# arpitbansal297/Cold-Diffusion-Models

Hardware: AMD Instinct MI355X
Metric: unet_train_imgs_per_sec (higher is better)
Workload: dtype f32 storage/accumulate; dense-conv GEMM operands bf16x3; 1 GPU; CelebA-128 denoising cold diffusion (BASELINE config 3): Unet(dim=64,(1,2,4,8),ch=3) @128x128, T=200, optimizer step = 2 micro-batches x 32 img (one fused forward / backward pass over all of them: same draws, same gradient sum) + Adam + EMA/10; per_gpu_batch=32, gradient_accumulate_every=2, parallelism=single

## Files before the change

### cold-diffusion-models_amd/csrc/k_conv_rowhalo.hip

```cpp
#include "cdf_conv_sp.h"

template <int W, int BN, int NS = 3, int NCH = 2, int BM = 256>
__global__ void __launch_bounds__(512, 1) conv_igemm_rowhalo_stream_kernel(SpxArgs a) {
    constexpr int WM = BM / 64, WN = 8 / WM, NW = 8, BK = 32, RE = CDF_SP_RE, MT = BM / WM / 32, NB = 3;
    static_assert(BM == 256 && WM * WN == 8 && MT == 2, "8 waves (4 x 2) of 64-row tiles");
    static_assert(NCH % 2 == 0, "an even number of tap-row groups per tile returns the pipeline to row buffer 0");
    using L = RowHaloLayout<W, BN, BM>;
    using Segs = typename L::Segs;
    constexpr int EROWS = L::EROWS, CP = L::CP;
    constexpr int TH = L::TH, HW2 = L::HW2, RH = L::RH;
    constexpr int TAG = Segs::PER_WAVE;
    constexpr int NT = BN / WN / 32;
    constexpr int SB = BN / 16 / NW;
    static_assert(SB * NW * 16 == BN || BN == 64, "B tile must split into 16-row segments");
    constexpr int SBI = BN == 64 ? 1 : SB;
    constexpr int PLANE_A = L::PLANE_A, PLANE_B = L::PLANE_B;
    CDF_DYN_SMEM(smem_raw);
    unsigned short* smem = (unsigned short*)smem_raw;
    float* const cs = (float*)(smem + L::OFF_CS);

    const int tid = threadIdx.x, lane = tid & 63, wave = __builtin_amdgcn_readfirstlane(tid >> 6);
    const int wm = wave / WN, wn = wave % WN;
    const int M = a.B * a.QH * a.QW;
    const int tiles_n = (a.Cout + BN - 1) / BN, tiles_m = M / BM, ntiles = tiles_m * tiles_n;
    const CdfPhase& ph = a.ph[0];
    const int tpi = a.H / TH;

    const int srow = cdf_dma_row(lane), q8 = cdf_dma_col(lane);
    int a_seg[TAG], a_ry[TAG], a_x[TAG];
#pragma unroll
    for (int q = 0; q < TAG; ++q) {
        const int g = a_seg[q] = Segs::seg(wave, q);
        const int r = g * 16 + srow;
        a_ry[q] = r < RH ? r / HW2 : -(1 << 20);
        a_x[q] = r - (r / HW2) * HW2 - 1;
    }
    auto fetch_a = [&](int img, int y0, int c, int dy, int buf) {
        unsigned short* base = smem + L::a_off(buf);
#pragma unroll
        for (int q = 0; q < TAG; ++q) {
            const int y = y0 + a_ry[q] + dy;
            const bool ok = img >= 0 && (unsigned)y < (unsigned)a.H && (unsigned)a_x[q] < (unsigned)W;
            const size_t off = ((size_t)(((ok ? img : 0) * a.H + (ok ? y : 0)) * W + (ok ? a_x[q] : 0))) * (unsigned)a.ldx + (unsigned)(c * BK + q8);
            unsigned short* seg = base + a_seg[q] * 16 * RE;
            CDF_GLDS16_K(ok ? a.x_hi + off : a.zero, seg);
            if constexpr (NS == 3) CDF_GLDS16_K(ok ? a.x_lo + off : a.zero, seg + PLANE_A);
        }
    };
    auto fetch_b = [&](int tile_n, int c, int wi, int stage) {
        unsigned short* st = smem + L::b_off(stage);
#pragma unroll
        for (int p = 0; p < SBI; ++p) {
            const int seg = BN == 64 ? (wave & 3) : wave * SB + p;
            const size_t woff = cdf_w_off(wi, a.Cout, cdf_w_row(tile_n * BN + seg * 16 + srow, a.Cout), a.ldk, c * BK + q8);
            CDF_GLDS16_K(a.w_hi + woff, st + seg * 16 * RE);
            if constexpr (NS == 3) CDF_GLDS16_K(a.w_lo + woff, st + PLANE_B + seg * 16 * RE);
        }
    };
    constexpr int NPL = NS == 3 ? 2 : 1;
    constexpr int PB = NPL * SBI, PAG = NPL * TAG;

    const int half = lane >> 5, l31 = lane & 31;
    int row0[MT];
#pragma unroll
    for (int i = 0; i < MT; ++i) {
        const int pix = wm * (BM / WM) + i * 32 + l31;
        const int py = pix / W, px = pix - py * W;
        row0[i] = py * HW2 + px + 1;
    }
    const bool late = a.dephase != 0 && wave >= NW / 2;

    auto tile_pos = [&](int v, int& img, int& y0, int& tn, int& tm) {
        if (v < ntiles) {
            const int tile = cdf_xcd_order(v, ntiles);
            tm = tile / tiles_n;
            tn = tile - tm * tiles_n;
            img = tm / tpi;
            y0 = (tm - img * tpi) * TH;
        } else {
            img = -1; y0 = 0; tn = 0; tm = 0;
        }
    };
    int img, y0, tile_n, tile_m;
    int v = blockIdx.x;
    tile_pos(v, img, y0, tile_n, tile_m);
    const bool fast_epi = cdf_epi_tile_ok<BM, BN>(a, M) && cdf_epi_family_ok(a.epi, NS == 1);
    fetch_a(img, y0, 0, ph.dy[0], 0);
    fetch_b(tile_n, 0, ph.wi[0], 0);
    fetch_b(tile_n, 0, ph.wi[1], 1);
    CDF_WAIT_DMA_LEAVE(PB);
    CDF_LDS_BARRIER();

    while (img >= 0) {
        int img_n, y0_n, tile_n_n, tile_m_n;
        tile_pos(v + gridDim.x, img_n, y0_n, tile_n_n, tile_m_n);
        f32x16_t acc[MT][NT];
        cdf_acc_zero(acc);
        bf16x8_v ah[2][MT], al[2][MT], bh[2][NT], bl[2][NT];
        if (late) cdf_frag_zero(ah, al, bh, bl);
        auto mma_frags = [&]() { cdf_mma_tile<NS, MT, NT>(acc, ah, al, bh, bl); };
        int row0t[MT], l31t = l31;
#pragma unroll
        for (int i = 0; i < MT; ++i) row0t[i] = row0[i];
#ifndef CDF_EMU
#pragma unroll
        for (int i = 0; i < MT; ++i) asm volatile("" : "+v"(row0t[i]));
        asm volatile("" : "+v"(l31t));
#endif
        const int swbt = (l31t >> 2) & 3;
#pragma unroll
        for (int g = 0; g < 3; ++g) {
#pragma unroll
            for (int c = 0; c < NCH; ++c) {
#pragma unroll
                for (int i3 = 0; i3 < 3; ++i3) {
                    const int t = 3 * g + i3;
                    const int step = (g * NCH + c) * 3 + i3;
                    const int par = (g * NCH + c) & 1, rd = step % NB;
                    {
                        const int s2 = step + 2, gc2 = (s2 / 3) % (3 * NCH);
                        const bool over = s2 >= 9 * NCH;
                        const int g2 = gc2 / NCH, c2 = gc2 - g2 * NCH;
                        fetch_b(over ? tile_n_n : tile_n, c2, ph.wi[3 * g2 + s2 % 3], s2 % NB);
                    }
                    if (i3 == 0) {
                        const bool lastc = c + 1 == NCH, over = lastc && g == 2;
                        const int nc = lastc ? 0 : c + 1, ng = over ? 0 : (lastc ? g + 1 : g);
                        fetch_a(over ? img_n : img, over ? y0_n : y0, nc, ph.dy[3 * ng], par ^ 1);
                    }
                    int sa_e = L::a_off(par), sb_e = L::b_off(rd);
#ifndef CDF_EMU
                    asm volatile("" : "+s"(sa_e), "+s"(sb_e));
#endif
                    const unsigned short* sa = smem + sa_e;
                    const unsigned short* sb = smem + sb_e;
                    const int dx = ph.dx[t];
                    auto read_frags = [&]() {
#pragma unroll
                        for (int ks = 0; ks < 2; ++ks) {
                            cdf_read_frags_halo<NS, PLANE_A>(ah[ks], al[ks], sa, ks, half, row0t, dx);
                            cdf_read_frags<NS, PLANE_B>(bh[ks], bl[ks], sb, ks, half, wn * (BN / WN) + l31t, swbt);
                        }
                    };
                    cdf_dephased_step(late, read_frags, mma_frags);
                    if (i3 <= 1)
                        CDF_WAIT_DMA_LEAVE(PB + PAG);
                    else
                        CDF_WAIT_DMA_LEAVE(PB);
                    CDF_LDS_BARRIER();
                }
            }
        }
        if (late) mma_frags();
        auto dump = [&](int hp) {
            if ((wm * 64) / EROWS == hp) {
                int base = (wm * 64 - hp * EROWS + 4 * half) * CP + wn * (BN / WN) + l31;
#ifndef CDF_EMU
                asm volatile("" : "+v"(base));
#endif
                cdf_acc_stage(cs + base, CP, 0, 0, acc, 0, 0);
            }
        };
        if (fast_epi) {
            const long long trow = (long long)tile_m * BM;
            cdf_epi_dispatch<NS == 1>(a.epi, [&](auto spec) {
                using E = cdf_epi_fast<BN, EROWS, 512, decltype(spec)>;
                f32x4_t q[E::NR], bs[2];
                cdf_epi_load_bias<BN, 512>(a, bs, trow, tile_n * BN, tid);
                E::load(a, q, trow, tile_n * BN, tid);
                dump(0);
                CDF_LDS_BARRIER();
                E::template finish<true>(a, q, bs, cs, trow, tile_n * BN, tid, trow + EROWS);
                CDF_LDS_BARRIER();
                dump(1);
                CDF_LDS_BARRIER();
                E::template finish<false>(a, q, bs, cs, trow + EROWS, tile_n * BN, tid);
                CDF_LDS_BARRIER();
            });
        } else {
#pragma unroll 1
            for (int hp = 0; hp < 2; ++hp) {
                dump(hp);
                CDF_LDS_BARRIER();
                cdf_epilogue_rows<BN, EROWS, 512>(a, ph, a.y, cs, tile_m * BM + hp * EROWS, tile_n * BN, M, tid, [](int p) { return p; });
                CDF_LDS_BARRIER();
            }
        }
        img = img_n; y0 = y0_n; tile_n = tile_n_n; tile_m = tile_m_n;
        v += gridDim.x;
    }
    CDF_WAIT_DMA_LEAVE(0);
}

template <int NS, int W, int BN>
static int launch_igemm_rowhalo_stream(const SpxArgs& a, int M, hipStream_t s, int reserve, CdfPlan* plan) {
    using L = RowHaloLayout<W, BN>;
    const int tiles = (M / 256) * cdf_cdiv(a.Cout, BN);
#ifdef CDF_EMU
    int ncu = cdf_num_cus() - reserve;
    if (ncu < 1) ncu = 1;
#else
    int ncu = cdf_num_cus() - (reserve + 7) / 8 * 8;
    if (ncu < 8) ncu = 8;
#endif
    const int grid = tiles < ncu ? tiles : ncu;
    if (plan) return cdf_plan_set(plan, CDF_FORM_ROWHALO, 256, BN, a.Cin == 64 ? 2 : 4, 1, W, tiles, grid);
    if (a.Cin == 64)
        CDF_LAUNCH_LDS((conv_igemm_rowhalo_stream_kernel<W, BN, NS, 2>), dim3(grid), dim3(512), L::bytes, s, a);
    else
        CDF_LAUNCH_LDS((conv_igemm_rowhalo_stream_kernel<W, BN, NS, 4>), dim3(grid), dim3(512), L::bytes, s, a);
    return cdf_check_launch("conv_igemm_rowhalo_stream");
}


template <int NS>
static int launch_rowhalo_ns(int W, bool n64, const SpxArgs& a, int M, hipStream_t s, int reserve, CdfPlan* plan) {
#define CDF_ROWHALO_CASE(WW) \
    if (W == WW) return n64 ? launch_igemm_rowhalo_stream<NS, WW, 64>(a, M, s, reserve, plan) : launch_igemm_rowhalo_stream<NS, WW, 128>(a, M, s, reserve, plan);
    CDF_ROWHALO_CASE(128)
#ifdef CDF_EMU
    CDF_ROWHALO_CASE(64) CDF_ROWHALO_CASE(32) CDF_ROWHALO_CASE(16)
#endif
#undef CDF_ROWHALO_CASE
    return CDF_E_UNSUPPORTED;
}

int cdf_launch_igemm_rowhalo(int ns, int W, bool n64, const SpxArgs& a, int M, hipStream_t s, int reserve, CdfPlan* plan) {
    return ns == 3 ? launch_rowhalo_ns<3>(W, n64, a, M, s, reserve, plan) : launch_rowhalo_ns<1>(W, n64, a, M, s, reserve, plan);
}
```

### cold-diffusion-models_amd/csrc/k_conv_spx.hip

```cpp
#include "cdf_conv_sp.h"

template <int BM, int BN, int WM, int WN, int NSTAGE, int OCC = 512 / (64 * WM * WN), int NS = 3>
__global__ void __launch_bounds__(64 * WM * WN, OCC) conv_igemm_spx_kernel(SpxArgs a) {
    constexpr int BK = 32, RE = CDF_SP_RE, NW = WM * WN;
    constexpr int MT = BM / WM / 32, NT = BN / WN / 32;
    constexpr int SA = BM / 16 / NW, SB = BN / 16 / NW;
    static_assert(SA >= 1 && SB >= 1 && SA * NW * 16 == BM && SB * NW * 16 == BN, "tile must split into 16-row segments per wave");
    using L = SpxLayout<BM, BN, NSTAGE>;
    constexpr int PLANE_A = L::PLANE_A, PLANE_B = L::PLANE_B, STAGE = L::STAGE;
    CDF_DYN_SMEM(smem_raw);
    unsigned short* smem = (unsigned short*)smem_raw;

    const int tid = threadIdx.x, lane = tid & 63, wave = __builtin_amdgcn_readfirstlane(tid >> 6);
    const int wm = wave / WN, wn = wave % WN;
    const int M = a.B * a.QH * a.QW;
    const int tiles_n = (a.Cout + BN - 1) / BN, tiles_m = (M + BM - 1) / BM;
    const int tile = cdf_xcd_order(blockIdx.x, tiles_m * tiles_n);
    const int tile_m = tile / tiles_n, tile_n = tile - tile_m * tiles_n;
    const CdfPhase& ph = a.ph[blockIdx.y];

    const int srow = cdf_dma_row(lane), q8 = cdf_dma_col(lane);
    int a_iy0[SA], a_ix0[SA], b_row[SB];
    unsigned a_pix[SA];
#pragma unroll
    for (int p = 0; p < SA; ++p) {
        const int m = tile_m * BM + (wave * SA + p) * 16 + srow;
        if (m < M) {
            const int qx = m % a.QW, t2 = m / a.QW;
            a_iy0[p] = (t2 % a.QH) * a.is;
            a_ix0[p] = qx * a.is;
            a_pix[p] = (unsigned)(((t2 / a.QH) * a.H + a_iy0[p]) * a.W + a_ix0[p]);
        } else {
            a_iy0[p] = -(1 << 28);
            a_ix0[p] = 0;
            a_pix[p] = 0;
        }
    }
#pragma unroll
    for (int p = 0; p < SB; ++p) {
        b_row[p] = cdf_w_row(tile_n * BN + (wave * SB + p) * 16 + srow, a.Cout);
    }
    const int nchunks = (a.Cin + BK - 1) / BK;
    const int ntaps_blk = a.ksplit > 1 ? ph.ntaps / a.ksplit : ph.ntaps;
    const int tap_lo = a.ksplit > 1 ? (int)blockIdx.z * ntaps_blk : 0;
    const int niter = ntaps_blk * nchunks;

    int* tap_lds = (int*)(smem + L::OFF_TAPS);
    if (tid <= CDF_MAX_TAPS) {
        int src = tid + tap_lo;
        if (src > CDF_MAX_TAPS) src = CDF_MAX_TAPS;
        if (a.taprot && tid < 9) {
            const int slot = tid / 3, kx = tid - 3 * slot;
#pragma unroll
            for (int g = 0; g < 3; ++g) {
                const int r = (tile_m + (int)ph.dy[3 * g]) % 3;
                if ((r < 0 ? r + 3 : r) == slot) src = 3 * g + kx;
            }
        }
        tap_lds[tid] = src < ph.ntaps ? (ph.dy[src] & 0xFF) | ((ph.dx[src] & 0xFF) << 8) | ((ph.wi[src] & 0xFF) << 16) : 0;
    }
    CDF_LDS_BARRIER();

    const unsigned short* pa_hi[SA];
    const unsigned short* pa_lo[SA];
    const unsigned short* pb_hi[SB];
    const unsigned short* pb_lo[SB];
    int a_inc[SA];
    const bool ragged = (a.Cin & (BK - 1)) != 0;
    auto retap = [&](int tap) {
        const int tc = tap_lds[tap];
        const int dy = (int)(signed char)(tc & 0xFF), dx = (int)(signed char)((tc >> 8) & 0xFF), wi = (tc >> 16) & 0xFF;
        const int tap_pix = dy * a.W + dx;
#pragma unroll
        for (int p = 0; p < SA; ++p) {
            const unsigned iy = (unsigned)(a_iy0[p] + dy), ix = (unsigned)(a_ix0[p] + dx);
            const bool ok = iy < (unsigned)a.H && ix < (unsigned)a.W && q8 < a.Cin;
            const size_t off = (size_t)(a_pix[p] + (unsigned)tap_pix) * (unsigned)a.ldx + (unsigned)q8;
            pa_hi[p] = ok ? a.x_hi + off : a.zero;
            pa_lo[p] = ok ? a.x_lo + off : a.zero;
            a_inc[p] = ok ? BK : 0;
        }
#pragma unroll
        for (int p = 0; p < SB; ++p) {
            const size_t woff = cdf_w_off(wi, a.Cout, b_row[p], a.ldk, q8);
            pb_hi[p] = a.w_hi + woff;
            pb_lo[p] = a.w_lo + woff;
        }
    };
    int tap = 0, c0 = 0, issued = 0;
    retap(0);
    auto fetch = [&](int buf) {
        unsigned short* st = smem + buf * STAGE;
        const bool cok = !ragged || (c0 + q8) < a.Cin;
#pragma unroll
        for (int p = 0; p < SA; ++p) {
            unsigned short* seg = st + (wave * SA + p) * 16 * RE;
            CDF_GLDS16(cok ? pa_hi[p] : a.zero, seg);
            if constexpr (NS == 3) CDF_GLDS16(cok ? pa_lo[p] : a.zero, seg + PLANE_A);
        }
#pragma unroll
        for (int p = 0; p < SB; ++p) {
            unsigned short* seg = st + L::OFF_B + (wave * SB + p) * 16 * RE;
            CDF_GLDS16(pb_hi[p], seg);
            if constexpr (NS == 3) CDF_GLDS16(pb_lo[p], seg + PLANE_B);
        }
        const bool more = issued + 1 < niter;
        issued += more ? 1 : 0;
        if (more) {
            c0 += BK;
            if (c0 >= a.Cin) {
                c0 = 0;
                ++tap;
                retap(tap);
            } else {
#pragma unroll
                for (int p = 0; p < SA; ++p) {
                    pa_hi[p] += a_inc[p];
                    pa_lo[p] += a_inc[p];
                }
#pragma unroll
                for (int p = 0; p < SB; ++p) {
                    pb_hi[p] += BK;
                    pb_lo[p] += BK;
                }
            }
        }
    };

    f32x16_t acc[MT][NT];
    cdf_acc_zero(acc);

    const int half = lane >> 5, l31 = lane & 31;
    const int sw = (l31 >> 2) & 3;
    constexpr int PIECES = (NS == 3 ? 2 : 1) * (SA + SB);
    int fbuf = 0;
    if (niter > 0) {
#pragma unroll
        for (int d = 0; d < NSTAGE - 1; ++d) {
            fetch(fbuf);
            fbuf = fbuf + 1 == NSTAGE ? 0 : fbuf + 1;
        }
    }
    CDF_WAIT_DMA_LEAVE((NSTAGE - 2) * PIECES);
    CDF_LDS_BARRIER();
    int buf = 0;
    bf16x8_v ah[2][MT], al[2][MT], bh[2][NT], bl[2][NT];
    const bool late = a.dephase != 0 && NW == 8 && wave >= 4;
    if (late) cdf_frag_zero(ah, al, bh, bl);
    auto fetch_read = [&]() {
        fetch(fbuf);
        fbuf = fbuf + 1 == NSTAGE ? 0 : fbuf + 1;
        const unsigned short* sa = smem + buf * STAGE;
        const unsigned short* sb = sa + L::OFF_B;
        buf = buf + 1 == NSTAGE ? 0 : buf + 1;
#pragma unroll
        for (int ks = 0; ks < 2; ++ks) {
            cdf_read_frags<NS, PLANE_A>(ah[ks], al[ks], sa, ks, half, wm * (BM / WM) + l31, sw);
            cdf_read_frags<NS, PLANE_B>(bh[ks], bl[ks], sb, ks, half, wn * (BN / WN) + l31, sw);
        }
    };
    auto mma_frags = [&]() { cdf_mma_tile<NS, MT, NT>(acc, ah, al, bh, bl); };
    for (int it = 0; it < niter; ++it) {
        cdf_dephased_step(late, fetch_read, mma_frags);
        CDF_WAIT_DMA_LEAVE((NSTAGE - 2) * PIECES);
        CDF_LDS_BARRIER();
    }
    if (late) mma_frags();
    CDF_WAIT_DMA_LEAVE(0);
    CDF_LDS_BARRIER();

    if (a.ksplit > 1) {
        RawEpiArgs r;
        r.Cout = a.Cout; r.vec = (a.Cout & 3) == 0 ? 1 : 0; r.os = 1; r.QH = 1; r.QW = 1; r.OH = 1; r.OW = 1; r.ldy = a.ks_ld;
        r.ldp = r.ldm = r.ldr = r.ld_sbias = r.ld_ys = 0; r.act = 0; r.mul_mode = 0; r.accumulate = 0;
        r.bias = nullptr; r.sbias = nullptr; r.pre = nullptr; r.mul = nullptr; r.res = nullptr; r.ys_hi = nullptr; r.ys_lo = nullptr; r.io_bf = 0;
        float* cs = (float*)smem_raw;
        cdf_acc_stage(cs, BN + 8, wm * (BM / WM), wn * (BN / WN), acc, half, l31);
        __syncthreads();
        cdf_epilogue_rows<BN, BM, 64 * WM * WN>(r, ph, a.ks_ws + (size_t)blockIdx.z * M * a.ks_ld, cs, tile_m * BM, tile_n * BN, M, tid,
                                                [](int p) { return p; });
        return;
    }
    cdf_sp_epilogue<BM, BN, WM, WN, NS == 1>(a, ph, acc, (float*)smem_raw, tile_m, tile_n, M, tid);
}

template <int BN>
__global__ void __launch_bounds__(256) conv_splitk_finish_kernel(SpxArgs a) {
    constexpr int BM = 16, CP = BN + 8;
    __shared__ __attribute__((aligned(16))) float cs[BM * CP];
    const int tid = threadIdx.x;
    const int M = a.B * a.QH * a.QW;
    const int tiles_n = (a.Cout + BN - 1) / BN;
    const int tile_m = blockIdx.x / tiles_n, tile_n = blockIdx.x - tile_m * tiles_n;
    constexpr int V = BN / 4;
    const size_t zs = (size_t)M * a.ks_ld;
    for (int e = tid; e < BM * V; e += 256) {
        const int r = e / V, c4 = (e - r * V) * 4;
        const int m = tile_m * BM + r, n = tile_n * BN + c4;
        const bool ok = m < M && n < a.ks_ld;
        const float* p = a.ks_ws + (ok ? (size_t)m * a.ks_ld + n : 0);
        float4 v[CDF_MAX_TAPS];
#pragma unroll
        for (int z = 0; z < CDF_MAX_TAPS; ++z) v[z] = *(const float4*)(p + (z < a.ksplit ? z : 0) * zs);
        float4 sum = make_float4(0.f, 0.f, 0.f, 0.f);
#pragma unroll
        for (int z = 0; z < CDF_MAX_TAPS; ++z)
            if (z < a.ksplit) { sum.x += v[z].x; sum.y += v[z].y; sum.z += v[z].z; sum.w += v[z].w; }
        *(float4*)(cs + r * CP + c4) = ok ? sum : make_float4(0.f, 0.f, 0.f, 0.f);
    }
    __syncthreads();
    cdf_epilogue_rows<BN, BM, 256>(a, a.ph[0], a.y, cs, tile_m * BM, tile_n * BN, M, tid, [](int p) { return p; });
}

extern "C" int cdf_gemm_tuning_default(cdf_gemm_tuning* t) {
    CDF_REQUIRE(t, "cdf_gemm_tuning_default: null pointer");
    *t = kTuneDefault;
    return 0;
}

template <int NS, int BM, int BN, int WM, int WN, int NSTAGE, int OCC = 512 / (64 * WM * WN)>
static int launch_igemm_spx(const SpxArgs& a, int M, hipStream_t s, CdfPlan* plan) {
    using L = SpxLayout<BM, BN, NSTAGE>;
    const int tiles = cdf_cdiv(M, BM) * cdf_cdiv(a.Cout, BN);
    if (plan) return cdf_plan_set(plan, CDF_FORM_SPX, BM, BN, NSTAGE, a.ksplit > 1 ? a.ksplit : 1, 0, tiles, (long long)tiles * a.nphase * (a.ksplit > 1 ? a.ksplit : 1));
    CDF_LAUNCH_LDS((conv_igemm_spx_kernel<BM, BN, WM, WN, NSTAGE, OCC, NS>), dim3(tiles, a.nphase, a.ksplit > 1 ? a.ksplit : 1), dim3(64 * WM * WN), L::bytes, s, a);
    if (a.ksplit > 1) {
        const int ftiles = cdf_cdiv(M, 16) * cdf_cdiv(a.Cout, BN);
        if (BN == 64) CDF_LAUNCH((conv_splitk_finish_kernel<64>), dim3(ftiles), dim3(256), 0, s, a);
        else CDF_LAUNCH((conv_splitk_finish_kernel<128>), dim3(ftiles), dim3(256), 0, s, a);
    }
    return cdf_check_launch("conv_igemm_spx");
}

static int spx_ksplit(int M, int Cout, int nphase, int ntaps, const cdf_gemm_tuning& T) {
    if (!T.splitk || !T.deep || nphase != 1 || (ntaps != 9 && ntaps != 16)) return 1;
    const bool n64 = Cout <= 64;
    const long long tiles128 = (long long)cdf_cdiv(M, 128) * cdf_cdiv(Cout, n64 ? 64 : 128);
    const long long tiles64 = (long long)cdf_cdiv(M, 64) * cdf_cdiv(Cout, n64 ? 64 : 128);
    if (tiles128 >= 384 || tiles64 > 128) return 1;
    for (int ks = 2; ks <= ntaps; ++ks)
        if (ntaps % ks == 0 && tiles64 * ks >= 192) return ks;
    return ntaps;
}
extern "C" int cdf_conv_gemm_bf16x_ksplit(int M, int Cout, int nphase, int ntaps, const cdf_gemm_tuning* tune) { return spx_ksplit(M, Cout, nphase, ntaps, *cdf_tune(tune)); }

template <int NS>
static int dispatch_gemm_bf16x(SpxArgs& a, long long ks_ws_floats, const cdf_gemm_tuning& T, hipStream_t s, int* bm_out = nullptr, CdfPlan* plan = nullptr) {
    const int B = a.B, H = a.H, W = a.W, Cin = a.Cin, Cout = a.Cout, QH = a.QH, QW = a.QW, os = a.os, is = a.is, nphase = a.nphase;
    const int M = B * QH * QW;
    const bool n64 = T.tile_bn ? T.tile_bn == 64 : Cout <= 64;
    const long long tiles128 = (long long)cdf_cdiv(M, 128) * cdf_cdiv(Cout, n64 ? 64 : 128) * nphase;
    bool m64 = tiles128 < 384;
    bool m256 = !n64 && tiles128 >= 1024 && T.max_bm != 128;
    if (T.tile_bm) { m64 = T.tile_bm == 64; m256 = T.tile_bm == 256 && !n64; }
    bool is3x3 = nphase == 1 && is == 1 && os == 1 && a.ph[0].ntaps == 9 && a.ph[0].oy == 0 && a.ph[0].ox == 0;
    if (is3x3) {
        int seen = 0;
        for (int g = 0; g < 3; ++g) {
            const int dy = a.ph[0].dy[3 * g];
            is3x3 = is3x3 && a.ph[0].dy[3 * g + 1] == dy && a.ph[0].dy[3 * g + 2] == dy && dy >= -1 && dy <= 1;
            seen |= 1 << (dy + 1);
        }
        is3x3 = is3x3 && seen == 7;
    }
    const bool rot_ok = is3x3;
    const int bm = m256 ? 256 : (m64 ? 64 : 128);
    a.taprot = rot_ok && QW == bm;
    a.dephase = T.dephase;
    if (T.halo && is3x3 && !T.tile_bm && QW == W && QH == H && Cin % 32 == 0 && Cin >= 64 && M % 128 == 0) {
        const bool n64_in = n64;
        int dxs = 0;
        for (int t = 0; t < 9; ++t) dxs |= 1 << (a.ph[0].dx[t] + 1);
        const bool dx_ok = dxs == 7;
        const bool n64 = n64_in || (T.small_n64 && !T.tile_bn && Cout > 64 && Cout % 64 == 0 && (long long)(M / 128) * cdf_cdiv(Cout, 128) < 176);
        const long long tiles = (long long)(M / 128) * cdf_cdiv(Cout, n64 ? 64 : 128);
        if (dx_ok && M % 256 == 0 && (T.rowhalo_stream & 1) && (Cin == 64 || Cin == 128) &&
            ((T.halo & 64) || ((T.halo & 32) && W == 128 && !n64 && (long long)(M / 256) * cdf_cdiv(Cout, 128) >= 256))) {
            if ((W == 128 || W == 64 || W == 32 || W == 16) && H % (256 / W) == 0) {
                const int rc = cdf_launch_igemm_rowhalo(NS, W, n64, a, M, s, T.resident_reserve, plan);
                if (rc != CDF_E_UNSUPPORTED) return rc;
            }
        }
        if (dx_ok && tiles >= (T.halo_min_tiles > 0 ? T.halo_min_tiles : 1)) {
            if ((W == 128 || W == 64 || W == 32 || W == 16) && (T.halo & (W / 16)) && H % (128 / W) == 0 && (W < 128 || n64 || (T.halo & 16))) {
                const bool bm256 = (W <= 64 || n64) && T.halo_bm != 128 && H % (256 / W) == 0 && M % 256 == 0 &&
                                   (T.halo_bm == 256 || (long long)(M / 256) * cdf_cdiv(Cout, n64 ? 64 : 128) >= 256);
                if (bm_out) *bm_out = bm256 ? 256 : 128;
                return cdf_launch_igemm_halo(NS, W, n64, bm256 ? 256 : 128, a, M, s, plan);
            }
        }
    }
    if (bm_out) *bm_out = bm;
    if (m256) return launch_igemm_spx<NS, 256, 128, 4, 2, 3>(a, M, s, plan);
    const long long tiles64 = (long long)cdf_cdiv(M, 64) * cdf_cdiv(Cout, n64 ? 64 : 128) * nphase;
    if (m64 && tiles64 <= 256 && T.deep) {
        const int ks = spx_ksplit(M, Cout, nphase, a.ph[0].ntaps, T);
        if (ks > 1 && a.ks_ws && ks_ws_floats >= (long long)ks * M * ((Cout + 3) / 4 * 4)) {
            a.ksplit = ks;
            a.ks_ld = (Cout + 3) / 4 * 4;
            a.taprot = 0;
        } else {
            a.ksplit = 1;
        }
        if (n64) return launch_igemm_spx<NS, 64, 64, 2, 2, 6, 1>(a, M, s, plan);
        return launch_igemm_spx<NS, 64, 128, 2, 2, 6, 1>(a, M, s, plan);
    }
    if (n64) return m64 ? launch_igemm_spx<NS, 64, 64, 2, 2, 2>(a, M, s, plan) : launch_igemm_spx<NS, 128, 64, 2, 2, 2>(a, M, s, plan);
    if (m64) return launch_igemm_spx<NS, 64, 128, 2, 2, 2>(a, M, s, plan);
    return launch_igemm_spx<NS, 128, 128, 2, 2, 2>(a, M, s, plan);
}

extern "C" int cdf_conv_gemm_bf16x_io(const void* x_hi, const void* x_lo, int ldx, const void* zero, const void* w_hi, const void* w_lo,
                                      int ldk, float* y, int ldy, int B, int H, int W, int Cin, int OH, int OW, int Cout, int QH, int QW,
                                      int os, int is, int nphase, const int* phase_desc, const float* bias, const float* sbias,
                                      int ld_sbias, const void* res, int ldr, void* pre, int ldp, const void* mul, int ldm, int act,
                                      int mul_mode, int accumulate, int io_bf16, void* y_hi, void* y_lo, int ld_ys, float* ws,
                                      long long ws_floats, const cdf_gemm_tuning* tune, void* stream);

extern "C" int cdf_conv_gemm_bf16x(const void* x_hi, const void* x_lo, int ldx, const void* zero, const void* w_hi, const void* w_lo,
                                   int ldk, float* y, int ldy, int B, int H, int W, int Cin, int OH, int OW, int Cout, int QH, int QW,
                                   int os, int is, int nphase, const int* phase_desc, const float* bias, const float* sbias,
                                   int ld_sbias, const float* res, int ldr, float* pre, int ldp, const float* mul, int ldm, int act,
                                   int mul_mode, int accumulate, void* y_hi, void* y_lo, int ld_ys, float* ws, long long ws_floats,
                                   const cdf_gemm_tuning* tune, void* stream) {
    return cdf_conv_gemm_bf16x_io(x_hi, x_lo, ldx, zero, w_hi, w_lo, ldk, y, ldy, B, H, W, Cin, OH, OW, Cout, QH, QW, os, is, nphase, phase_desc,
                                  bias, sbias, ld_sbias, res, ldr, pre, ldp, mul, ldm, act, mul_mode, accumulate, 0, y_hi, y_lo, ld_ys, ws,
                                  ws_floats, tune, stream);
}

extern "C" int cdf_conv_gemm_bf16x_io(const void* x_hi, const void* x_lo, int ldx, const void* zero, const void* w_hi, const void* w_lo,
                                      int ldk, float* y, int ldy, int B, int H, int W, int Cin, int OH, int OW, int Cout, int QH, int QW,
                                      int os, int is, int nphase, const int* phase_desc, const float* bias, const float* sbias,
                                      int ld_sbias, const void* res_, int ldr, void* pre_, int ldp, const void* mul_, int ldm, int act,
                                      int mul_mode, int accumulate, int io_bf16, void* y_hi, void* y_lo, int ld_ys, float* ws,
                                      long long ws_floats, const cdf_gemm_tuning* tune, void* stream) {
    const float* res = (const float*)res_;
    float* pre = (float*)pre_;
    const float* mul = (const float*)mul_;
    CDF_REQUIRE((io_bf16 & ~15) == 0, "cdf_conv_gemm_bf16x_io: io_bf16 has unknown bits (%d)", io_bf16);
    CDF_REQUIRE(!(io_bf16 & CDF_IO_PRE_GRAD) || (pre_ && (act == 1 || act == 2)), "cdf_conv_gemm_bf16x_io: CDF_IO_PRE_GRAD needs a pre tensor and act = GELU / SiLU");
    CDF_REQUIRE(x_hi && zero && w_hi && (y || (y_hi && !accumulate)), "cdf_conv_gemm_bf16x: null pointer");
    CDF_TUNE_CHECK(tune, "cdf_conv_gemm_bf16x");
    CDF_REQUIRE(!ws || (((uintptr_t)ws) & 15) == 0, "cdf_conv_gemm_bf16x: the split-K workspace must be 16-byte aligned");
    CDF_REQUIRE((x_lo != nullptr) == (w_lo != nullptr), "cdf_conv_gemm_bf16x: pass both lo planes (split precision, 3 MFMAs per product) or neither (single-pass bf16)");
    CDF_REQUIRE((!y_hi && !y_lo) || (y_hi && ld_ys % 4 == 0 && ld_ys >= Cout && Cout % 4 == 0 && ((((uintptr_t)y_hi) | ((uintptr_t)y_lo)) & 7) == 0),
                "cdf_conv_gemm_bf16x: output planes need Cout %% 4 == 0, ld_ys %% 4 == 0, 8-byte alignment (y_lo optional: hi-only planes)");
    CDF_REQUIRE(((((uintptr_t)x_hi) | ((uintptr_t)x_lo) | ((uintptr_t)zero) | ((uintptr_t)w_hi) | ((uintptr_t)w_lo)) & 15) == 0, "cdf_conv_gemm_bf16x: operands must be 16B aligned");
    CDF_REQUIRE(ldx % 8 == 0 && Cin % 8 == 0 && ldx >= Cin && ldk % 32 == 0 && ldk >= Cin, "cdf_conv_gemm_bf16x: Cin and pitches must be multiples of 8 (ldk of 32)");
    CDF_REQUIRE(nphase >= 1 && nphase <= 4 && phase_desc && (!y || ldy >= Cout), "cdf_conv_gemm_bf16x: bad geometry");
    CDF_REQUIRE(!mul_mode || mul, "cdf_conv_gemm_bf16x: mul_mode without mul tensor");
    SpxArgs a;
    a.x_hi = (const unsigned short*)x_hi; a.x_lo = (const unsigned short*)x_lo; a.zero = (const unsigned short*)zero;
    a.w_hi = (const unsigned short*)w_hi; a.w_lo = (const unsigned short*)w_lo; a.ldx = ldx; a.ldk = ldk;
    cdf_fill_gemm_common(a, y, ldy, bias, sbias, ld_sbias, res, ldr, pre, ldp, mul, ldm, B, H, W, Cin, OH, OW, Cout, QH, QW, os, is, nphase, act, mul_mode,
                         accumulate, y_hi, y_lo, ld_ys, io_bf16);
    cdf_clear_epi(a);
    if (cdf_tune(tune)->epilogue) a.epi = cdf_epi_select(a);
    CDF_REQUIRE(!y_hi || a.vec, "cdf_conv_gemm_bf16x: split output planes need the vectorised epilogue (aligned pointers, pitches %% 4)");
    CDF_REQUIRE(!(io_bf16 & 7) || a.vec, "cdf_conv_gemm_bf16x_io: bf16 epilogue operands need the vectorised epilogue (16-byte-aligned pointers, pitches %% 4, Cout %% 4)");
    int rc = cdf_fill_phases(a.ph, nphase, phase_desc, "cdf_conv_gemm_bf16x");
    if (rc) return rc;
    a.ksplit = 1; a.ks_ws = ws; a.ks_ld = 0;
    return x_lo ? dispatch_gemm_bf16x<3>(a, ws ? ws_floats : 0, *cdf_tune(tune), CDF_S)
                : dispatch_gemm_bf16x<1>(a, ws ? ws_floats : 0, *cdf_tune(tune), CDF_S);
}


extern "C" int cdf_conv_gemm_bf16x_lnbwd_ok(int B, int H, int W, int Cin, int Cout, int nphase, int ntaps) {
    const long long M = (long long)B * H * W;
    return (Cout == 64 || Cout == 128) && nphase == 1 && ntaps == 9 && M % 256 == 0 && M < (1ll << 31) && Cin % 32 == 0 && Cin >= 64;
}
static cdf_gemm_tuning lnbwd_tuning(const cdf_gemm_tuning* tune) {
    cdf_gemm_tuning T = *cdf_tune(tune);
    T.rowhalo_stream = 0; T.small_n64 = 0; T.tile_bn = 0; T.splitk = 0;
    return T;
}

extern "C" int cdf_conv_gemm_bf16x_form(int B, int H, int W, int Cin, int Cout, int QH, int QW, int os, int is, int nphase, const int* phase_desc,
                                        int ns, long long ws_floats, int lnbwd, const cdf_gemm_tuning* tune, int* tiles_grid) {
    CDF_REQUIRE(phase_desc && nphase >= 1 && nphase <= 4 && (ns == 1 || ns == 3) && B >= 1, "cdf_conv_gemm_bf16x_form: bad arguments");
    CDF_TUNE_CHECK(tune, "cdf_conv_gemm_bf16x_form");
    CDF_REQUIRE(!lnbwd || cdf_conv_gemm_bf16x_lnbwd_ok(B, H, W, Cin, Cout, nphase, phase_desc[2]), "cdf_conv_gemm_bf16x_form: not a geometry of cdf_conv_gemm_bf16x_lnbwd");
    SpxArgs a = {};
    cdf_fill_gemm_common(a, nullptr, 0, nullptr, nullptr, 0, nullptr, 0, nullptr, 0, nullptr, 0, B, H, W, Cin, 0, 0, Cout, QH, QW, os, is, nphase, 0, 0, 0, nullptr, nullptr, 0, 0);
    int rc = cdf_fill_phases(a.ph, nphase, phase_desc, "cdf_conv_gemm_bf16x_form");
    if (rc) return rc;
    static float ws_token;
    a.ksplit = 1; a.ks_ws = (ws_floats > 0 && !lnbwd) ? &ws_token : nullptr; a.ks_ld = 0;
    const cdf_gemm_tuning T = lnbwd ? lnbwd_tuning(tune) : *cdf_tune(tune);
    CdfPlan plan = {0, 0, 0};
    rc = ns == 3 ? dispatch_gemm_bf16x<3>(a, a.ks_ws ? ws_floats : 0, T, nullptr, nullptr, &plan)
                 : dispatch_gemm_bf16x<1>(a, a.ks_ws ? ws_floats : 0, T, nullptr, nullptr, &plan);
    if (rc) return rc;
    if (tiles_grid) { tiles_grid[0] = plan.tiles; tiles_grid[1] = plan.grid; }
    return plan.code;
}

extern "C" int cdf_conv_gemm_bf16x_lnbwd(const void* x_hi, const void* x_lo, int ldx, const void* zero, const void* w_hi, const void* w_lo, int ldk,
                                         int B, int H, int W, int Cin, int Cout, const int* phase_desc, const float* ln_x, int ld_lnx,
                                         const float* ln_mean, const float* ln_rstd, const float* ln_g, float* dh, int lddh, float* dg, float* db,
                                         float* part, const cdf_gemm_tuning* tune, void* stream) {
    CDF_REQUIRE(x_hi && zero && w_hi && phase_desc && ln_x && ln_mean && ln_rstd && ln_g && dh && dg && db && part, "cdf_conv_gemm_bf16x_lnbwd: null pointer");
    CDF_TUNE_CHECK(tune, "cdf_conv_gemm_bf16x_lnbwd");
    CDF_REQUIRE((x_lo != nullptr) == (w_lo != nullptr), "cdf_conv_gemm_bf16x_lnbwd: pass both lo planes or neither");
    CDF_REQUIRE(cdf_conv_gemm_bf16x_lnbwd_ok(B, H, W, Cin, Cout, 1, phase_desc[2]), "cdf_conv_gemm_bf16x_lnbwd: needs a 3 x 3 stride-1 layer with 64 or 128 output channels, B*H*W %% 256 == 0");
    CDF_REQUIRE(((((uintptr_t)x_hi) | ((uintptr_t)x_lo) | ((uintptr_t)zero) | ((uintptr_t)w_hi) | ((uintptr_t)w_lo) | ((uintptr_t)ln_x) | ((uintptr_t)ln_g) | ((uintptr_t)dh)) & 15) == 0 &&
                ldx % 8 == 0 && ldx >= Cin && ldk % 32 == 0 && ldk >= Cin && ld_lnx % 4 == 0 && ld_lnx >= Cout && lddh % 4 == 0 && lddh >= Cout,
                "cdf_conv_gemm_bf16x_lnbwd: alignment / pitches");
    SpxArgs a;
    a.x_hi = (const unsigned short*)x_hi; a.x_lo = (const unsigned short*)x_lo; a.zero = (const unsigned short*)zero;
    a.w_hi = (const unsigned short*)w_hi; a.w_lo = (const unsigned short*)w_lo; a.ldx = ldx; a.ldk = ldk;
    cdf_fill_gemm_common(a, dh, lddh, ln_g, nullptr, 0, nullptr, 0, nullptr, 0, nullptr, 0, B, H, W, Cin, H, W, Cout, H, W, 1, 1, 1, 0, 0, 0, nullptr, nullptr, 0, 0);
    a.vec = 1;
    a.epi = CDF_EPI_LNBWD;
    a.ln_x = ln_x; a.ln_mean = ln_mean; a.ln_rstd = ln_rstd; a.ln_part = part; a.ld_lnx = ld_lnx;
    int rc = cdf_fill_phases(a.ph, 1, phase_desc, "cdf_conv_gemm_bf16x_lnbwd");
    if (rc) return rc;
    a.ksplit = 1; a.ks_ws = nullptr; a.ks_ld = 0;
    const cdf_gemm_tuning T = lnbwd_tuning(tune);
    int bm = 0;
    rc = x_lo ? dispatch_gemm_bf16x<3>(a, 0, T, CDF_S, &bm) : dispatch_gemm_bf16x<1>(a, 0, T, CDF_S, &bm);
    if (rc) return rc;
    CDF_REQUIRE(bm == 64 || bm == 128 || bm == 256, "cdf_conv_gemm_bf16x_lnbwd: the dispatcher reported no row tile");
    return cdf_norm_param_reduce(part, (int)((long long)B * H * W / bm), Cout, dg, db, 1, stream);
}
```

Baseline: 1333 img/s.

## Use 16x16 MFMA tiles for bf16x3 conv kernels in rowhalo and spx paths

```diff
diff --git a/cold-diffusion-models_amd/csrc/k_conv_rowhalo.hip b/cold-diffusion-models_amd/csrc/k_conv_rowhalo.hip
--- a/cold-diffusion-models_amd/csrc/k_conv_rowhalo.hip
+++ b/cold-diffusion-models_amd/csrc/k_conv_rowhalo.hip
@@ -1,10 +1,16 @@
 #include "cdf_conv_sp.h"
+
+constexpr int cdf_rowhalo_mfma(int W, int BN, int NS, int NCH) {
+    (void)W;
+    return NS == 3 && BN == 128 && NCH == 2 ? 16 : 32;
+}
 
 template <int W, int BN, int NS = 3, int NCH = 2, int BM = 256>
 __global__ void __launch_bounds__(512, 1) conv_igemm_rowhalo_stream_kernel(SpxArgs a) {
     constexpr int WM = BM / 64, WN = 8 / WM, NW = 8, BK = 32, RE = CDF_SP_RE, MT = BM / WM / 32, NB = 3;
     static_assert(BM == 256 && WM * WN == 8 && MT == 2, "8 waves (4 x 2) of 64-row tiles");
     static_assert(NCH % 2 == 0, "an even number of tap-row groups per tile returns the pipeline to row buffer 0");
+    constexpr int MF = cdf_rowhalo_mfma(W, BN, NS, NCH);
     using L = RowHaloLayout<W, BN, BM>;
     using Segs = typename L::Segs;
     constexpr int EROWS = L::EROWS, CP = L::CP;
@@ -26,7 +32,7 @@
     const CdfPhase& ph = a.ph[0];
     const int tpi = a.H / TH;
 
-    const int srow = cdf_dma_row(lane), q8 = cdf_dma_col(lane);
+    const int srow = cdf_dma_row(lane), q8 = cdf_dma_col<MF>(lane);
     int a_seg[TAG], a_ry[TAG], a_x[TAG];
 #pragma unroll
     for (int q = 0; q < TAG; ++q) {
@@ -61,13 +67,17 @@
     constexpr int PB = NPL * SBI, PAG = NPL * TAG;
 
     const int half = lane >> 5, l31 = lane & 31;
-    int row0[MT];
-#pragma unroll
-    for (int i = 0; i < MT; ++i) {
-        const int pix = wm * (BM / WM) + i * 32 + l31;
-        const int py = pix / W, px = pix - py * W;
-        row0[i] = py * HW2 + px + 1;
-    }
+    constexpr int NF = MF == 16 ? 2 : 1;
+    const int lrow = MF == 16 ? lane & 15 : l31, kblk = MF == 16 ? lane >> 4 : half;
+    int row0[NF][MT];
+#pragma unroll
+    for (int f = 0; f < NF; ++f)
+#pragma unroll
+        for (int i = 0; i < MT; ++i) {
+            const int pix = wm * (BM / WM) + i * 32 + f * 16 + lrow;
+            const int py = pix / W, px = pix - py * W;
+            row0[f][i] = py * HW2 + px + 1;
+        }
     const bool late = a.dephase != 0 && wave >= NW / 2;
 
     auto tile_pos = [&](int v, int& img, int& y0, int& tn, int& tm) {
@@ -94,20 +104,24 @@
     while (img >= 0) {
         int img_n, y0_n, tile_n_n, tile_m_n;
         tile_pos(v + gridDim.x, img_n, y0_n, tile_n_n, tile_m_n);
-        f32x16_t acc[MT][NT];
+        typename cdf_acc_of<MF>::type acc[MT][NT];
         cdf_acc_zero(acc);
         bf16x8_v ah[2][MT], al[2][MT], bh[2][NT], bl[2][NT];
         if (late) cdf_frag_zero(ah, al, bh, bl);
         auto mma_frags = [&]() { cdf_mma_tile<NS, MT, NT>(acc, ah, al, bh, bl); };
-        int row0t[MT], l31t = l31;
-#pragma unroll
-        for (int i = 0; i < MT; ++i) row0t[i] = row0[i];
+        int row0t[NF][MT], lrowt = lrow;
+#pragma unroll
+        for (int f = 0; f < NF; ++f)
+#pragma unroll
+            for (int i = 0; i < MT; ++i) row0t[f][i] = row0[f][i];
 #ifndef CDF_EMU
 #pragma unroll
-        for (int i = 0; i < MT; ++i) asm volatile("" : "+v"(row0t[i]));
-        asm volatile("" : "+v"(l31t));
-#endif
-        const int swbt = (l31t >> 2) & 3;
+        for (int f = 0; f < NF; ++f)
+#pragma unroll
+            for (int i = 0; i < MT; ++i) asm volatile("" : "+v"(row0t[f][i]));
+        asm volatile("" : "+v"(lrowt));
+#endif
+        const int swbt = cdf_swz<MF>(lrowt);
 #pragma unroll
         for (int g = 0; g < 3; ++g) {
 #pragma unroll
@@ -138,8 +152,8 @@
                     auto read_frags = [&]() {
 #pragma unroll
                         for (int ks = 0; ks < 2; ++ks) {
-                            cdf_read_frags_halo<NS, PLANE_A>(ah[ks], al[ks], sa, ks, half, row0t, dx);
-                            cdf_read_frags<NS, PLANE_B>(bh[ks], bl[ks], sb, ks, half, wn * (BN / WN) + l31t, swbt);
+                            cdf_read_frags_halo<NS, PLANE_A, MT, MF>(ah[ks], al[ks], sa, ks, kblk, row0t[MF == 16 ? ks : 0], dx);
+                            cdf_read_frags<NS, PLANE_B, NT, MF>(bh[ks], bl[ks], sb, ks, kblk, wn * (BN / WN) + (MF == 16 ? 16 * ks : 0) + lrowt, swbt);
                         }
                     };
                     cdf_dephased_step(late, read_frags, mma_frags);
@@ -154,7 +168,7 @@
         if (late) mma_frags();
         auto dump = [&](int hp) {
             if ((wm * 64) / EROWS == hp) {
-                int base = (wm * 64 - hp * EROWS + 4 * half) * CP + wn * (BN / WN) + l31;
+                int base = (wm * 64 - hp * EROWS + 4 * kblk) * CP + wn * (BN / WN) + lrow;
 #ifndef CDF_EMU
                 asm volatile("" : "+v"(base));
 #endif
diff --git a/cold-diffusion-models_amd/csrc/k_conv_spx.hip b/cold-diffusion-models_amd/csrc/k_conv_spx.hip
--- a/cold-diffusion-models_amd/csrc/k_conv_spx.hip
+++ b/cold-diffusion-models_amd/csrc/k_conv_spx.hip
@@ -1,4 +1,8 @@
 #include "cdf_conv_sp.h"
+
+constexpr int cdf_spx_mfma(int BM, int BN, int NSTAGE, int NS) {
+    return NS == 3 && NSTAGE <= 3 && !(BM == 64 && BN == 64) ? 16 : 32;
+}
 
 template <int BM, int BN, int WM, int WN, int NSTAGE, int OCC = 512 / (64 * WM * WN), int NS = 3>
 __global__ void __launch_bounds__(64 * WM * WN, OCC) conv_igemm_spx_kernel(SpxArgs a) {
@@ -8,6 +12,7 @@
     static_assert(SA >= 1 && SB >= 1 && SA * NW * 16 == BM && SB * NW * 16 == BN, "tile must split into 16-row segments per wave");
     using L = SpxLayout<BM, BN, NSTAGE>;
     constexpr int PLANE_A = L::PLANE_A, PLANE_B = L::PLANE_B, STAGE = L::STAGE;
+    constexpr int MF = cdf_spx_mfma(BM, BN, NSTAGE, NS);
     CDF_DYN_SMEM(smem_raw);
     unsigned short* smem = (unsigned short*)smem_raw;
 
@@ -19,7 +24,7 @@
     const int tile_m = tile / tiles_n, tile_n = tile - tile_m * tiles_n;
     const CdfPhase& ph = a.ph[blockIdx.y];
 
-    const int srow = cdf_dma_row(lane), q8 = cdf_dma_col(lane);
+    const int srow = cdf_dma_row(lane), q8 = cdf_dma_col<MF>(lane);
     int a_iy0[SA], a_ix0[SA], b_row[SB];
     unsigned a_pix[SA];
 #pragma unroll
@@ -127,11 +132,12 @@
         }
     };
 
-    f32x16_t acc[MT][NT];
+    typename cdf_acc_of<MF>::type acc[MT][NT];
     cdf_acc_zero(acc);
 
     const int half = lane >> 5, l31 = lane & 31;
-    const int sw = (l31 >> 2) & 3;
+    const int lrow = MF == 16 ? lane & 15 : l31, kblk = MF == 16 ? lane >> 4 : half;
+    const int sw = cdf_swz<MF>(lrow);
     constexpr int PIECES = (NS == 3 ? 2 : 1) * (SA + SB);
     int fbuf = 0;
     if (niter > 0) {
@@ -155,8 +161,8 @@
         buf = buf + 1 == NSTAGE ? 0 : buf + 1;
 #pragma unroll
         for (int ks = 0; ks < 2; ++ks) {
-            cdf_read_frags<NS, PLANE_A>(ah[ks], al[ks], sa, ks, half, wm * (BM / WM) + l31, sw);
-            cdf_read_frags<NS, PLANE_B>(bh[ks], bl[ks], sb, ks, half, wn * (BN / WN) + l31, sw);
+            cdf_read_frags<NS, PLANE_A, MT, MF>(ah[ks], al[ks], sa, ks, kblk, wm * (BM / WM) + (MF == 16 ? 16 * ks : 0) + lrow, sw);
+            cdf_read_frags<NS, PLANE_B, NT, MF>(bh[ks], bl[ks], sb, ks, kblk, wn * (BN / WN) + (MF == 16 ? 16 * ks : 0) + lrow, sw);
         }
     };
     auto mma_frags = [&]() { cdf_mma_tile<NS, MT, NT>(acc, ah, al, bh, bl); };
```

Result: no change. 1338 img/s (median of 6 runs) (+0.4%).
